# tomerlieber/doc-agents

Measured on AMD Instinct MI355X. Metric: QA queries/sec + p50 cache-miss latency; docs/min ingest at 1/2/4/8 MI355X, higher is better.
Workload: dtype bf16

## Files before the change

### docagents_amd/ops/csrc/gemm8p.hip

```cpp
#include "gemm.h"

#include <cstdlib>
#include <type_traits>

typedef __attribute__((address_space(3))) void* lds_ptr_t;

namespace {
constexpr int BN = 256;
constexpr int HALF_B = 16384;
constexpr int SROW = 64 * 2 + 16;
}

template <int N>
__device__ __forceinline__ void vmcnt() {
  asm volatile("s_waitcnt vmcnt(%0)" ::"n"(N) : "memory");
}

template <int EPI, int BM, typename T = BF16T, bool PERSIST = false>
__global__ void __launch_bounds__(512)
gemm8p_kernel(GemmArgs p) {
  static_assert(BM == 256 || BM == 128, "BM");
  constexpr int HALF_A = BM / 2 * 128;
  constexpr int OFF_A0 = 0, OFF_A1 = HALF_A, OFF_B0 = 2 * HALF_A, OFF_B1 = 2 * HALF_A + HALF_B;
  constexpr int BUF = 2 * HALF_A + 2 * HALF_B;
  constexpr int STAGING = 8 * (BM / 2) * SROW;
  constexpr int SMEM = (2 * BUF > STAGING) ? 2 * BUF : STAGING;
  constexpr int MI = BM / 64;
  constexpr int QR = BM / 4;
  constexpr int NA = BM / 128;
  constexpr int CNT_AB = 2 * NA + 4;
  __shared__ __attribute__((aligned(16))) char smem[SMEM];
  const int tid = threadIdx.x, lane = tid & 63;
  const int wid = __builtin_amdgcn_readfirstlane(tid >> 6);
  const int wg = wid >> 2, wn = wid & 3;
  const int fr = lane & 15, fg = lane >> 4;

  const int ntm = (p.M + BM - 1) / BM, ntn = (p.N + BN - 1) / BN, ntiles = ntm * ntn;
  const int GROUP = p.group > 0 ? p.group : 4;
  auto tile_of = [&](int id, int& m0_, int& n0_) __attribute__((always_inline)) {
    const int t = xcd_remap(id, ntiles);
    const int gid = t / (GROUP * ntn);
    const int first_m = gid * GROUP;
    const int gsz = min(ntm - first_m, GROUP);
    const int tin = t % (GROUP * ntn);
    m0_ = (first_m + tin % gsz) * BM;
    n0_ = (tin / gsz) * BN;
  };
  int id = blockIdx.x, m0, n0;
  tile_of(id, m0, n0);

  __amdgpu_buffer_rsrc_t rsa, rsw;
  unsigned aoffs[2][2], boffs[2][2];
  auto sources = [&](int m0_, int n0_) __attribute__((always_inline)) {
    int sl = lane;
    if constexpr (PERSIST) asm volatile("" : "+v"(sl));
    rsa = __builtin_amdgcn_make_buffer_rsrc(
        (void*)((const char*)p.A + (size_t)m0_ * p.lda * 2), (short)0, 0x7ffffff0, 0x00020000);
    rsw = __builtin_amdgcn_make_buffer_rsrc(
        (void*)((const char*)p.W + (size_t)n0_ * p.K * 2), (short)0, 0x7ffffff0, 0x00020000);
#pragma unroll
    for (int j = 0; j < NA; ++j) {
      const int r = (wid * NA + j) * 8 + (sl >> 3);
      const int c = (sl & 7) ^ ((r >> 1) & 7);
#pragma unroll
      for (int h = 0; h < 2; ++h)
        aoffs[h][j] = (unsigned)(min(m0_ + h * (BM / 2) + r, p.M - 1) - m0_) * (unsigned)(p.lda * 2) + c * 16;
    }
#pragma unroll
    for (int j = 0; j < 2; ++j) {
      const int r = (wid * 2 + j) * 8 + (sl >> 3);
      const int c = (sl & 7) ^ ((r >> 1) & 7);
#pragma unroll
      for (int h = 0; h < 2; ++h)
        boffs[h][j] = (unsigned)(min(n0_ + h * 128 + r, p.N - 1) - n0_) * (unsigned)(p.K * 2) + c * 16;
    }
  };
#define ISSUE_A(H, KT, B)                                                                               \
  do {                                                                                                  \
    char* d_ = smem + (B) * BUF + ((H) ? OFF_A1 : OFF_A0) + wid * NA * 1024;                            \
    _Pragma("unroll") for (int j_ = 0; j_ < NA; ++j_)                                                   \
      __builtin_amdgcn_raw_ptr_buffer_load_lds(rsa, (lds_ptr_t)(d_ + j_ * 1024), 16, aoffs[H][j_], (KT) * 128, 0, 0); \
  } while (0)
#define ISSUE_B(H, KT, B)                                                                               \
  do {                                                                                                  \
    char* d_ = smem + (B) * BUF + ((H) ? OFF_B1 : OFF_B0) + wid * 2048;                                 \
    _Pragma("unroll") for (int j_ = 0; j_ < 2; ++j_)                                                    \
      __builtin_amdgcn_raw_ptr_buffer_load_lds(rsw, (lds_ptr_t)(d_ + j_ * 1024), 16, boffs[H][j_], (KT) * 128, 0, 0); \
  } while (0)
  auto prologue = [&]() __attribute__((always_inline)) {
    ISSUE_A(0, 0, 0); ISSUE_B(0, 0, 0); ISSUE_B(1, 0, 0); ISSUE_A(1, 0, 0);
    ISSUE_A(0, 1, 1); ISSUE_B(0, 1, 1); ISSUE_B(1, 1, 1);
  };

  int aoff[2], boff[2];
#pragma unroll
  for (int kk = 0; kk < 2; ++kk) {
    const int cs = ((kk * 4 + fg) ^ (fr >> 1)) << 4;
    aoff[kk] = (wg * QR + fr) * 128 + cs;
    boff[kk] = (wn * 32 + fr) * 128 + cs;
  }

  f32x4_t acc[2][2][MI][2];
  bf16x8_t ra[2][MI], rb0[2][2], rb1[2][2];
  auto read_a = [&](const char* base) __attribute__((always_inline)) {
#pragma unroll
    for (int kk = 0; kk < 2; ++kk)
#pragma unroll
      for (int i = 0; i < MI; ++i) ra[kk][i] = *(const bf16x8_t*)(base + aoff[kk] + i * 2048);
  };
  auto read_b = [&](bf16x8_t (&rb)[2][2], const char* base) __attribute__((always_inline)) {
#pragma unroll
    for (int kk = 0; kk < 2; ++kk)
#pragma unroll
      for (int j = 0; j < 2; ++j) rb[kk][j] = *(const bf16x8_t*)(base + boff[kk] + j * 2048);
  };
  auto bar = [&]() __attribute__((always_inline)) {
    __builtin_amdgcn_sched_barrier(0);
    __builtin_amdgcn_s_barrier();
    __builtin_amdgcn_sched_barrier(0);
  };
  auto lgkm0 = [&]() __attribute__((always_inline)) {
    asm volatile("s_waitcnt lgkmcnt(0)" ::: "memory");
    __builtin_amdgcn_sched_barrier(0);
  };
  auto quad = [&](auto ih_t, auto jh_t, bf16x8_t (&rb)[2][2]) __attribute__((always_inline)) {
    constexpr int IH = decltype(ih_t)::value, JH = decltype(jh_t)::value;
#pragma unroll
    for (int kk = 0; kk < 2; ++kk)
#pragma unroll
      for (int i = 0; i < MI; ++i)
#pragma unroll
        for (int j = 0; j < 2; ++j) acc[IH][JH][i][j] = T::mma16(rb[kk][j], ra[kk][i], acc[IH][JH][i][j]);
  };
  using I0 = std::integral_constant<int, 0>;
  using I1 = std::integral_constant<int, 1>;

  auto ktile = [&](int kt, auto fill_tag, auto next_tag, auto x_tag) __attribute__((always_inline)) {
    constexpr bool FILL = decltype(fill_tag)::value;
    constexpr bool NEXT = decltype(next_tag)::value;
    constexpr int X = decltype(x_tag)::value;
    const int b = kt & 1;
    const char* base = smem + b * BUF;
    read_a(base + OFF_A0);
    read_b(rb0, base + OFF_B0);
    read_b(rb1, base + OFF_B1);
    if constexpr (NEXT) { ISSUE_A(1, kt + 1, b ^ 1); vmcnt<CNT_AB + X>(); }
    else { vmcnt<0>(); }
    lgkm0();
    bar();
    __builtin_amdgcn_s_setprio(1);
    quad(I0{}, I0{}, rb0);
    quad(I0{}, I1{}, rb1);
    __builtin_amdgcn_s_setprio(0);
    bar();
    read_a(base + OFF_A1);
    if constexpr (FILL) { ISSUE_A(0, kt + 2, b); ISSUE_B(0, kt + 2, b); ISSUE_B(1, kt + 2, b); vmcnt<CNT_AB + X>(); }
    else if constexpr (NEXT) { vmcnt<NA + X>(); }
    lgkm0();
    bar();
    __builtin_amdgcn_s_setprio(1);
    quad(I1{}, I1{}, rb1);
    quad(I1{}, I0{}, rb0);
    __builtin_amdgcn_s_setprio(0);
    bar();
  };
  using T_ = std::true_type;
  using F_ = std::false_type;
  const int nk = p.K / 64;

  constexpr bool SW = (EPI == EPI_SWIGLU);
  constexpr int HC = SW ? 16 : 32;
  constexpr int CPR = 2 * HC / 8;
  constexpr int RPI = 64 / CPR;
  constexpr int NI = (BM / 2) / RPI;
  constexpr int NB = NI < 8 ? NI : 8;
  const int ncols = SW ? p.N / 2 : p.N;

  constexpr int XS = (PERSIST && EPI != EPI_ROPE) ? NI : 0;
  using X0 = std::integral_constant<int, 0>;
  using XN = std::integral_constant<int, XS>;

  sources(m0, n0);
  prologue();
  bool first = true;
  for (;;) {
    if (first) vmcnt<CNT_AB>();
    else vmcnt<CNT_AB + XS>();
    bar();
    if (wg) bar();
#pragma unroll
    for (int a = 0; a < 2; ++a)
#pragma unroll
      for (int b = 0; b < 2; ++b)
#pragma unroll
        for (int i = 0; i < MI; ++i)
#pragma unroll
          for (int j = 0; j < 2; ++j) acc[a][b][i][j] = f32x4_t{0.f, 0.f, 0.f, 0.f};
    if (nk > 2) {
      if (first) ktile(0, T_{}, T_{}, X0{});
      else ktile(0, T_{}, T_{}, XN{});
      for (int kt = 1; kt < nk - 2; ++kt) ktile(kt, T_{}, T_{}, X0{});
      ktile(nk - 2, F_{}, T_{}, X0{});
    } else {
      if (first) ktile(0, F_{}, T_{}, X0{});
      else ktile(0, F_{}, T_{}, XN{});
    }
    ktile(nk - 1, F_{}, F_{}, X0{});
    first = false;
    if (!wg) bar();
    __syncthreads();

    int el = lane;
    if constexpr (PERSIST) asm volatile("" : "+v"(el));
    const int efr = el & 15, efg = el >> 4;
    const int ch = el % CPR;
    const int jh = ch / (HC / 8);
    const int cc = (ch % (HC / 8)) * 8;
    const int lr0 = el / CPR;
    char* st = smem + wid * (BM / 2) * SROW;
    if constexpr (EPI == EPI_SWIGLU) {
#pragma unroll
      for (int ih = 0; ih < 2; ++ih)
#pragma unroll
        for (int jh_ = 0; jh_ < 2; ++jh_)
#pragma unroll
          for (int i = 0; i < MI; ++i) {
            float v[4];
#pragma unroll
            for (int q = 0; q < 4; ++q) v[q] = silu(acc[ih][jh_][i][0][q]) * acc[ih][jh_][i][1][q];
            *(u32x2_t*)(st + (ih * QR + i * 16 + efr) * SROW + (jh_ * 16 + efg * 4) * 2) =
                u32x2_t{T::pack2(v[0], v[1]), T::pack2(v[2], v[3])};
          }
    } else {
      float bv[2][2][4] = {};
      if (p.bias) {
#pragma unroll
        for (int jh_ = 0; jh_ < 2; ++jh_)
#pragma unroll
          for (int j = 0; j < 2; ++j)
#pragma unroll
            for (int q = 0; q < 4; ++q) {
              const int gc = n0 + jh_ * 128 + wn * 32 + j * 16 + efg * 4 + q;
              bv[jh_][j][q] = gc < p.N ? T::to_f(p.bias[gc]) : 0.f;
            }
      }
#pragma unroll
      for (int ih = 0; ih < 2; ++ih)
#pragma unroll
        for (int jh_ = 0; jh_ < 2; ++jh_)
#pragma unroll
          for (int i = 0; i < MI; ++i)
#pragma unroll
            for (int j = 0; j < 2; ++j) {
              float v[4];
#pragma unroll
              for (int q = 0; q < 4; ++q) {
                v[q] = acc[ih][jh_][i][j][q] + bv[jh_][j][q];
                if constexpr (EPI == EPI_GELU) v[q] = gelu_erf(v[q]);
              }
              *(u32x2_t*)(st + (ih * QR + i * 16 + efr) * SROW + (jh_ * 32 + j * 16 + efg * 4) * 2) =
                  u32x2_t{T::pack2(v[0], v[1]), T::pack2(v[2], v[3])};
            }
    }
    __syncthreads();
    const int gcol = (SW ? n0 / 2 : n0) + jh * (SW ? 64 : 128) + wn * HC + cc;
    const bool col_ok = gcol < ncols;
    [[maybe_unused]] int rkind = 0, rhead = 0, rd0 = 0;
    if constexpr (EPI == EPI_ROPE) {
      const RopeArgs& R = p.rope;
      const int qw = R.H * R.D, kw = R.Hkv * R.D;
      rkind = gcol < qw ? 0 : (gcol < qw + kw ? 1 : 2);
      const int rel = gcol - (rkind == 0 ? 0 : (rkind == 1 ? qw : qw + kw));
      rhead = rel / R.D;
      rd0 = rel % R.D;
    }
    int gmv[NI];
    u32x4_t vv[NI];
    [[maybe_unused]] u32x4_t rr[EPI == EPI_RESID ? NI : 1];
    [[maybe_unused]] int psv[EPI == EPI_ROPE ? NI : 1], slv[EPI == EPI_ROPE ? NI : 1];
#pragma unroll
    for (int i = 0; i < NI; ++i) {
      const int lr = lr0 + i * RPI;
      gmv[i] = m0 + (lr / QR) * (BM / 2) + wg * QR + (lr % QR);
      const int gmc = min(gmv[i], p.M - 1);
      vv[i] = *(const u32x4_t*)(st + lr * SROW + (jh * HC + cc) * 2);
      if constexpr (EPI == EPI_RESID)
        rr[i] = *(const u32x4_t*)(p.resid + (size_t)gmc * p.ldr + (col_ok ? gcol : 0));
      if constexpr (EPI == EPI_ROPE) {
        psv[i] = p.rope.pos[gmc];
        slv[i] = p.rope.slot[gmc];
      }
    }
    [[maybe_unused]] __amdgpu_buffer_rsrc_t rsc;
    if constexpr (XS > 0)
      rsc = __builtin_amdgcn_make_buffer_rsrc((void*)(p.C + (size_t)m0 * p.ldc), (short)0,
                                              (int)min((long long)(p.M - m0) * p.ldc * 2, 0x7ffffff0ll), 0x00020000);
    const int nid = id + (int)gridDim.x;
    const bool more = PERSIST && nid < ntiles;
    int nm0 = 0, nn0 = 0;
    if constexpr (PERSIST) {
      lgkm0();
      bar();
      if (more) {
        tile_of(nid, nm0, nn0);
        sources(nm0, nn0);
        prologue();
      }
    }
#pragma unroll
    for (int i0 = 0; i0 < NI; i0 += NB) {
      if constexpr (EPI == EPI_ROPE) {
        const RopeArgs& R = p.rope;
        const int half = R.D / 2, i0c = rd0 / 2;
        f32x4_t c01[NB], c23[NB];
        if (rkind < 2) {
#pragma unroll
          for (int i = 0; i < NB; ++i) {
            const int ps = min(max(psv[i0 + i], 0), R.max_seq - 1);
            c01[i] = *(const f32x4_t*)(R.cs + ((size_t)ps * half + i0c) * 2);
            c23[i] = *(const f32x4_t*)(R.cs + ((size_t)ps * half + i0c) * 2 + 4);
          }
        }
#pragma unroll
        for (int i = 0; i < NB; ++i) {
          const int gm = gmv[i0 + i];
          if (gm >= p.M || !col_ok) continue;
          u32x4_t v = vv[i0 + i];
          const int ps = psv[i0 + i], sl = slv[i0 + i];
          DA_ASSERT(ps >= 0 && ps < R.max_seq && sl >= 0);
          if (rkind < 2) {
            const float ccs[4] = {c01[i][0], c01[i][2], c23[i][0], c23[i][2]};
            const float sns[4] = {c01[i][1], c01[i][3], c23[i][1], c23[i][3]};
#pragma unroll
            for (int e = 0; e < 4; ++e) {
              const float x1 = bf2f((bf16_t)(v[e] & 0xffff)), x2 = bf2f((bf16_t)(v[e] >> 16));
              const float o1 = x1 * ccs[e] - x2 * sns[e];
              const float o2 = x2 * ccs[e] + x1 * sns[e];
              v[e] = pack_bf2(o1, o2);
            }
          }
          if (rkind > 0) {
            bf16_t* cache = rkind == 1 ? R.kc : R.vc;
            *(u32x4_t*)(cache + (((size_t)sl * R.Hkv + rhead) * R.max_seq + ps) * R.D + rd0) = v;
            if (!R.kv_out) continue;
          }
          *(u32x4_t*)(p.C + (size_t)gm * p.ldc + gcol) = v;
        }
      } else {
#pragma unroll
        for (int i = 0; i < NB; ++i) {
          const int gm = gmv[i0 + i];
          if (XS == 0 && (gm >= p.M || !col_ok)) continue;
          u32x4_t v = vv[i0 + i];
          if constexpr (EPI == EPI_RESID) {
#pragma unroll
            for (int e = 0; e < 4; ++e) {
              const float lo = T::to_f((bf16_t)(v[e] & 0xffff)) + T::to_f((bf16_t)(rr[i0 + i][e] & 0xffff));
              const float hi = T::to_f((bf16_t)(v[e] >> 16)) + T::to_f((bf16_t)(rr[i0 + i][e] >> 16));
              v[e] = T::pack2(lo, hi);
            }
          }
          if constexpr (XS > 0) {
            const unsigned off = col_ok ? (unsigned)((gm - m0) * p.ldc + gcol) * 2u : 0x80000000u;
            __builtin_amdgcn_raw_buffer_store_b128(v, rsc, off, 0, 0);
          } else {
            *(u32x4_t*)(p.C + (size_t)gm * p.ldc + gcol) = v;
          }
        }
      }
    }
    if (!more) break;
    id = nid; m0 = nm0; n0 = nn0;
  }
#undef ISSUE_A
#undef ISSUE_B
}

static int num_cus() {
  static int cus = 0;
  if (cus <= 0) {
    int dev = 0;
    if (hipGetDevice(&dev) != hipSuccess ||
        hipDeviceGetAttribute(&cus, hipDeviceAttributeMultiprocessorCount, dev) != hipSuccess || cus <= 0)
      cus = 256;
  }
  return cus;
}

static int g_persist = -1;
static bool persist_on() {
  if (g_persist < 0) {
    const char* e = getenv("DA_GEMM8P_PERSIST");
    g_persist = (e && e[0] == '0') ? 0 : 1;
  }
  return g_persist == 1;
}

DA_EXPORT int da_gemm8p_persist(int on) {
  const int prev = persist_on() ? 1 : 0;
  if (on == 0 || on == 1) g_persist = on;
  return prev;
}

template <int EPI, int BM, typename T>
static void launch8p_epi(const GemmArgs& a, int ntiles, hipStream_t s) {
  const int cus = num_cus();
  if constexpr (EPI != EPI_ROPE) {
    if (persist_on() && ntiles > cus && cus >= 8) {
      gemm8p_kernel<EPI, BM, T, true><<<dim3(cus & ~7), dim3(512), 0, s>>>(a);
      return;
    }
  }
  gemm8p_kernel<EPI, BM, T, false><<<dim3(ntiles), dim3(512), 0, s>>>(a);
}

template <int BM>
static int launch8p(const GemmArgs& a0, int epi, hipStream_t s) {
  GemmArgs a = a0;
  if (a.group <= 0) a.group = 4;
  const int ntm = (a.M + BM - 1) / BM, ntn = (a.N + BN - 1) / BN;
  const int nt = ntm * ntn;
  if (epi >= 100) {
    switch (epi - 100) {
      case EPI_NONE: launch8p_epi<EPI_NONE, BM, F16T>(a, nt, s); break;
      case EPI_BIAS: launch8p_epi<EPI_BIAS, BM, F16T>(a, nt, s); break;
      case EPI_GELU: launch8p_epi<EPI_GELU, BM, F16T>(a, nt, s); break;
      case EPI_RESID: launch8p_epi<EPI_RESID, BM, F16T>(a, nt, s); break;
      default: return (int)hipErrorInvalidValue;
    }
    return (int)hipGetLastError();
  }
  switch (epi) {
    case EPI_NONE: launch8p_epi<EPI_NONE, BM, BF16T>(a, nt, s); break;
    case EPI_BIAS: launch8p_epi<EPI_BIAS, BM, BF16T>(a, nt, s); break;
    case EPI_GELU: launch8p_epi<EPI_GELU, BM, BF16T>(a, nt, s); break;
    case EPI_SWIGLU: launch8p_epi<EPI_SWIGLU, BM, BF16T>(a, nt, s); break;
    case EPI_RESID: launch8p_epi<EPI_RESID, BM, BF16T>(a, nt, s); break;
    case EPI_ROPE: launch8p_epi<EPI_ROPE, BM, BF16T>(a, nt, s); break;
    default: return (int)hipErrorInvalidValue;
  }
  return (int)hipGetLastError();
}

int launch_gemm8p(const GemmArgs& a, int epi, hipStream_t s, int bm) {
  if (a.K < 128 || a.K % 64) return (int)hipErrorInvalidValue;
  if ((size_t)bm * a.lda * 2 >= 0x7ffffff0ull || (size_t)256 * a.K * 2 >= 0x7ffffff0ull) return (int)hipErrorInvalidValue;
  return bm == 128 ? launch8p<128>(a, epi, s) : launch8p<256>(a, epi, s);
}

DA_EXPORT int da_gemm_f16(const void* A, int lda, const void* W, void* C, int ldc, const void* bias,
                          const void* resid, int ldr, int M, int N, int K, int epi, int bm, void* stream) {
  if (M < 1 || K % 64 || K < 128 || N % 8 || lda % 8 || ldc % 8) return (int)hipErrorInvalidValue;
  if (bm != 128 && bm != 256) return (int)hipErrorInvalidValue;
  if (epi != EPI_NONE && epi != EPI_BIAS && epi != EPI_GELU && epi != EPI_RESID) return (int)hipErrorInvalidValue;
  if (epi == EPI_RESID && (!resid || ldr % 8)) return (int)hipErrorInvalidValue;
  GemmArgs a{};
  a.A = (const bf16_t*)A; a.W = (const bf16_t*)W; a.C = (bf16_t*)C;
  a.bias = (const bf16_t*)bias; a.resid = (const bf16_t*)resid;
  a.M = M; a.N = N; a.K = K; a.lda = lda; a.ldc = ldc; a.ldr = ldr; a.k_per_split = K;
  return launch_gemm8p(a, 100 + epi, (hipStream_t)stream, bm);
}
```

Measured before the change: 36.21.

## Enable persistent scheduling for RoPE GEMM epilogue with per-tile row table

Extends the persistent-kernel path to the fused RoPE/KV-cache epilogue. Per-row position and slot lookups are loaded once per tile into an LDS row table holding the cos/sin offset and cache byte offset, instead of being gathered per lane. Column-kind dispatch is specialised at tile granularity, and output stores use buffer stores with out-of-range offsets. The next tile's prologue is issued in the middle of the RoPE epilogue so global loads overlap the epilogue. The change adds LDS usage and code complexity, plus a new restriction on max_seq*D size.

```diff
diff --git a/docagents_amd/ops/csrc/gemm8p.hip b/docagents_amd/ops/csrc/gemm8p.hip
--- a/docagents_amd/ops/csrc/gemm8p.hip
+++ b/docagents_amd/ops/csrc/gemm8p.hip
@@ -25,11 +25,12 @@
   constexpr int BUF = 2 * HALF_A + 2 * HALF_B;
   constexpr int STAGING = 8 * (BM / 2) * SROW;
   constexpr int SMEM = (2 * BUF > STAGING) ? 2 * BUF : STAGING;
+  constexpr int ROWTAB = EPI == EPI_ROPE ? BM * 16 : 0;
   constexpr int MI = BM / 64;
   constexpr int QR = BM / 4;
   constexpr int NA = BM / 128;
   constexpr int CNT_AB = 2 * NA + 4;
-  __shared__ __attribute__((aligned(16))) char smem[SMEM];
+  __shared__ __attribute__((aligned(16))) char smem[SMEM + ROWTAB];
   const int tid = threadIdx.x, lane = tid & 63;
   const int wid = __builtin_amdgcn_readfirstlane(tid >> 6);
   const int wg = wid >> 2, wn = wid & 3;
@@ -176,7 +177,7 @@
   constexpr int NB = NI < 8 ? NI : 8;
   const int ncols = SW ? p.N / 2 : p.N;
 
-  constexpr int XS = (PERSIST && EPI != EPI_ROPE) ? NI : 0;
+  constexpr int XS = PERSIST ? NI : 0;
   using X0 = std::integral_constant<int, 0>;
   using XN = std::integral_constant<int, XS>;
 
@@ -210,6 +211,16 @@
     if (!wg) bar();
     __syncthreads();
 
+    char* const rowtab = smem + SMEM;
+    [[maybe_unused]] int tps = 0, tsl = 0;
+    if constexpr (EPI == EPI_ROPE) {
+      if (wid < BM / 64) {
+        const int gmc = min(m0 + tid, p.M - 1);
+        tps = p.rope.pos[gmc];
+        tsl = p.rope.slot[gmc];
+      }
+    }
+
     int el = lane;
     if constexpr (PERSIST) asm volatile("" : "+v"(el));
     const int efr = el & 15, efg = el >> 4;
@@ -261,6 +272,15 @@
               *(u32x2_t*)(st + (ih * QR + i * 16 + efr) * SROW + (jh_ * 32 + j * 16 + efg * 4) * 2) =
                   u32x2_t{T::pack2(v[0], v[1]), T::pack2(v[2], v[3])};
             }
+    }
+    if constexpr (EPI == EPI_ROPE) {
+      if (wid < BM / 64) {
+        const RopeArgs& R = p.rope;
+        DA_ASSERT(tps >= 0 && tps < R.max_seq && tsl >= 0);
+        const unsigned cso = (unsigned)min(max(tps, 0), R.max_seq - 1) * (unsigned)(R.D * 4);
+        const size_t rb = (((size_t)tsl * R.Hkv) * R.max_seq + tps) * R.D * 2;
+        *(u32x4_t*)(rowtab + tid * 16) = u32x4_t{cso, 0u, (unsigned)rb, (unsigned)(rb >> 32)};
+      }
     }
     __syncthreads();
     const int gcol = (SW ? n0 / 2 : n0) + jh * (SW ? 64 : 128) + wn * HC + cc;
@@ -277,7 +297,6 @@
     int gmv[NI];
     u32x4_t vv[NI];
     [[maybe_unused]] u32x4_t rr[EPI == EPI_RESID ? NI : 1];
-    [[maybe_unused]] int psv[EPI == EPI_ROPE ? NI : 1], slv[EPI == EPI_ROPE ? NI : 1];
 #pragma unroll
     for (int i = 0; i < NI; ++i) {
       const int lr = lr0 + i * RPI;
@@ -286,67 +305,93 @@
       vv[i] = *(const u32x4_t*)(st + lr * SROW + (jh * HC + cc) * 2);
       if constexpr (EPI == EPI_RESID)
         rr[i] = *(const u32x4_t*)(p.resid + (size_t)gmc * p.ldr + (col_ok ? gcol : 0));
-      if constexpr (EPI == EPI_ROPE) {
-        psv[i] = p.rope.pos[gmc];
-        slv[i] = p.rope.slot[gmc];
-      }
     }
     [[maybe_unused]] __amdgpu_buffer_rsrc_t rsc;
-    if constexpr (XS > 0)
+    if constexpr (XS > 0 || EPI == EPI_ROPE)
       rsc = __builtin_amdgcn_make_buffer_rsrc((void*)(p.C + (size_t)m0 * p.ldc), (short)0,
                                               (int)min((long long)(p.M - m0) * p.ldc * 2, 0x7ffffff0ll), 0x00020000);
     const int nid = id + (int)gridDim.x;
     const bool more = PERSIST && nid < ntiles;
     int nm0 = 0, nn0 = 0;
-    if constexpr (PERSIST) {
-      lgkm0();
-      bar();
-      if (more) {
-        tile_of(nid, nm0, nn0);
-        sources(nm0, nn0);
-        prologue();
-      }
-    }
-#pragma unroll
-    for (int i0 = 0; i0 < NI; i0 += NB) {
-      if constexpr (EPI == EPI_ROPE) {
-        const RopeArgs& R = p.rope;
-        const int half = R.D / 2, i0c = rd0 / 2;
-        f32x4_t c01[NB], c23[NB];
-        if (rkind < 2) {
+#define HANDOFF()                                                                        \
+  do {                                                                                   \
+    if constexpr (PERSIST) {                                                             \
+      lgkm0();                                                                           \
+      bar();        \
+      if (more) {                                                                        \
+        tile_of(nid, nm0, nn0);                                                          \
+        sources(nm0, nn0);                                                               \
+        prologue();                                                                      \
+      }                                                                                  \
+    }                                                                                    \
+  } while (0)
+    if constexpr (EPI == EPI_ROPE) {
+      const RopeArgs& R = p.rope;
+      const int qw = R.H * R.D, kw = R.Hkv * R.D;
+      const int c0 = n0 + wn * HC;
+      const int mrem = p.M - m0;
+      const int tr0 = wg * QR + (lr0 & (RPI - 1));
+      auto trc = [](int i) { return (i * RPI / QR) * (BM / 2) + i * RPI % QR; };
+      static_assert(QR % RPI == 0, "a lane's rows keep their offset in the quadrant");
+      auto rope_store = [&](auto kind_tag) __attribute__((always_inline)) {
+        constexpr int KIND = decltype(kind_tag)::value;
+        const int rk = KIND == 3 ? rkind : KIND;
+        const unsigned csl = (unsigned)(rd0 / 2) * 8u;
+        char* const cl = (char*)(rk == 1 ? R.kc : R.vc) + ((size_t)rhead * R.max_seq * R.D + rd0) * 2;
+        const bool cst = KIND == 0 || KIND == 3 || R.kv_out;
+        const unsigned coff = (col_ok && (rk == 0 || R.kv_out)) ? (unsigned)(tr0 * p.ldc + gcol) * 2u : 0x80000000u;
+#pragma unroll
+        for (int i0 = 0; i0 < NI; i0 += NB) {
+          unsigned cso[NB];
+          unsigned long long rb[NB];
+          f32x4_t c01[NB], c23[NB];
 #pragma unroll
           for (int i = 0; i < NB; ++i) {
-            const int ps = min(max(psv[i0 + i], 0), R.max_seq - 1);
-            c01[i] = *(const f32x4_t*)(R.cs + ((size_t)ps * half + i0c) * 2);
-            c23[i] = *(const f32x4_t*)(R.cs + ((size_t)ps * half + i0c) * 2 + 4);
+            const char* e = rowtab + (tr0 + trc(i0 + i)) * 16;
+            if (KIND != 2) cso[i] = *(const unsigned*)e;
+            if (KIND != 0) rb[i] = *(const unsigned long long*)(e + 8);
+          }
+          if (KIND != 2 && rk < 2) {
+#pragma unroll
+            for (int i = 0; i < NB; ++i) {
+              const char* c = (const char*)R.cs + (cso[i] + csl);
+              c01[i] = *(const f32x4_t*)c;
+              c23[i] = *(const f32x4_t*)(c + 16);
+            }
+          }
+          if (i0 == 0) HANDOFF();
+#pragma unroll
+          for (int i = 0; i < NB; ++i) {
+            u32x4_t v = vv[i0 + i];
+            if (KIND != 2 && rk < 2) {
+              const float ccs[4] = {c01[i][0], c01[i][2], c23[i][0], c23[i][2]};
+              const float sns[4] = {c01[i][1], c01[i][3], c23[i][1], c23[i][3]};
+#pragma unroll
+              for (int e = 0; e < 4; ++e) {
+                const float x1 = bf2f((bf16_t)(v[e] & 0xffff)), x2 = bf2f((bf16_t)(v[e] >> 16));
+                const float o1 = x1 * ccs[e] - x2 * sns[e];
+                const float o2 = x2 * ccs[e] + x1 * sns[e];
+                v[e] = pack_bf2(o1, o2);
+              }
+            }
+            if (KIND != 0 && rk > 0 && col_ok && tr0 + trc(i0 + i) < mrem) *(u32x4_t*)(cl + rb[i]) = v;
+            if (cst) __builtin_amdgcn_raw_buffer_store_b128(v, rsc, coff + (unsigned)(trc(i0 + i) * p.ldc) * 2u, 0, 0);
           }
         }
-#pragma unroll
-        for (int i = 0; i < NB; ++i) {
-          const int gm = gmv[i0 + i];
-          if (gm >= p.M || !col_ok) continue;
-          u32x4_t v = vv[i0 + i];
-          const int ps = psv[i0 + i], sl = slv[i0 + i];
-          DA_ASSERT(ps >= 0 && ps < R.max_seq && sl >= 0);
-          if (rkind < 2) {
-            const float ccs[4] = {c01[i][0], c01[i][2], c23[i][0], c23[i][2]};
-            const float sns[4] = {c01[i][1], c01[i][3], c23[i][1], c23[i][3]};
-#pragma unroll
-            for (int e = 0; e < 4; ++e) {
-              const float x1 = bf2f((bf16_t)(v[e] & 0xffff)), x2 = bf2f((bf16_t)(v[e] >> 16));
-              const float o1 = x1 * ccs[e] - x2 * sns[e];
-              const float o2 = x2 * ccs[e] + x1 * sns[e];
-              v[e] = pack_bf2(o1, o2);
-            }
-          }
-          if (rkind > 0) {
-            bf16_t* cache = rkind == 1 ? R.kc : R.vc;
-            *(u32x4_t*)(cache + (((size_t)sl * R.Hkv + rhead) * R.max_seq + ps) * R.D + rd0) = v;
-            if (!R.kv_out) continue;
-          }
-          *(u32x4_t*)(p.C + (size_t)gm * p.ldc + gcol) = v;
-        }
-      } else {
+      };
+      using K0 = std::integral_constant<int, 0>;
+      using K1 = std::integral_constant<int, 1>;
+      using K2 = std::integral_constant<int, 2>;
+      using K3 = std::integral_constant<int, 3>;
+      if (c0 + 128 + HC <= qw) rope_store(K0{});
+      else if (c0 >= qw + kw) rope_store(K2{});
+      else if (c0 >= qw && c0 + 128 + HC <= qw + kw) rope_store(K1{});
+      else rope_store(K3{});
+      if constexpr (PERSIST) first = !(mrem >= BM && c0 < p.N);
+    } else {
+      HANDOFF();
+#pragma unroll
+      for (int i0 = 0; i0 < NI; i0 += NB) {
 #pragma unroll
         for (int i = 0; i < NB; ++i) {
           const int gm = gmv[i0 + i];
@@ -372,6 +417,7 @@
     if (!more) break;
     id = nid; m0 = nm0; n0 = nn0;
   }
+#undef HANDOFF
 #undef ISSUE_A
 #undef ISSUE_B
 }
@@ -405,11 +451,9 @@
 template <int EPI, int BM, typename T>
 static void launch8p_epi(const GemmArgs& a, int ntiles, hipStream_t s) {
   const int cus = num_cus();
-  if constexpr (EPI != EPI_ROPE) {
-    if (persist_on() && ntiles > cus && cus >= 8) {
-      gemm8p_kernel<EPI, BM, T, true><<<dim3(cus & ~7), dim3(512), 0, s>>>(a);
-      return;
-    }
+  if (persist_on() && ntiles > cus && cus >= 8) {
+    gemm8p_kernel<EPI, BM, T, true><<<dim3(cus & ~7), dim3(512), 0, s>>>(a);
+    return;
   }
   gemm8p_kernel<EPI, BM, T, false><<<dim3(ntiles), dim3(512), 0, s>>>(a);
 }
@@ -445,6 +489,7 @@
 int launch_gemm8p(const GemmArgs& a, int epi, hipStream_t s, int bm) {
   if (a.K < 128 || a.K % 64) return (int)hipErrorInvalidValue;
   if ((size_t)bm * a.lda * 2 >= 0x7ffffff0ull || (size_t)256 * a.K * 2 >= 0x7ffffff0ull) return (int)hipErrorInvalidValue;
+  if (epi == EPI_ROPE && (size_t)a.rope.max_seq * a.rope.D * 4 >= 0xffffffffull) return (int)hipErrorInvalidValue;
   return bm == 128 ? launch8p<128>(a, epi, s) : launch8p<256>(a, epi, s);
 }
 
```

Result: no change. 36.25 (median of 6 runs) (+0.1%).
